# aliabdelkader/FusionTransformer

Measured on AMD Instinct MI355X. Metric: frames/sec fwd+bwd (SemanticKITTI synth), whole job, higher is better.
Workload: dtype f32

## Files before the change

### fusiontransformer_amd/csrc/ftx_spconv.hip

```cpp
#include <cstring>
#include <cstdlib>
#include "ftx_common.h"
#include <rocprim/device/device_scan.hpp>
#include <rocprim/iterator/transform_iterator.hpp>

using namespace ftx;

typedef float f32x16 __attribute__((ext_vector_type(16)));

struct IsValid {
  __host__ __device__ int32_t operator()(int32_t v) const { return v >= 0 ? 1 : 0; }
};

extern "C" size_t ftx_kernel_map_count_workspace_bytes(int64_t n_out, int32_t k) {
  if (n_out <= 0 || k <= 0) return 256;
  size_t bytes = 0;
  const int32_t *in = nullptr;
  int32_t *out = nullptr;
  auto it = rocprim::make_transform_iterator(in, IsValid());
  if (rocprim::exclusive_scan(nullptr, bytes, it, out, 0, (size_t)(n_out * k), rocprim::plus<int32_t>()) != hipSuccess) return 0;
  return bytes + 256;
}

__global__ void koff_kernel(const int32_t *__restrict__ nbr, const int32_t *__restrict__ scan, int64_t n_out, int k, int32_t *__restrict__ koff) {
  int t = blockIdx.x * blockDim.x + threadIdx.x;
  if (t < k) koff[t] = scan[(int64_t)t * n_out];
  if (t == k) {
    int64_t last = (int64_t)k * n_out - 1;
    koff[k] = scan[last] + (nbr[last] >= 0 ? 1 : 0);
  }
}

extern "C" int ftx_kernel_map_count(const int32_t *nbr, int64_t n_out, int32_t k, int32_t *pos, int32_t *koff, void *workspace,
                                    size_t workspace_bytes, void *stream) {
  FTX_REQUIRE(n_out >= 0 && k >= 1, "ftx_kernel_map_count: bad size");
  FTX_REQUIRE(koff, "ftx_kernel_map_count: null koff");
  hipStream_t st = (hipStream_t)stream;
  if (n_out == 0) {
    if (hipMemsetAsync(koff, 0, sizeof(int32_t) * (k + 1), st) != hipSuccess) return check_launch("ftx_kernel_map_count memset");
    return FTX_OK;
  }
  FTX_REQUIRE(nbr && pos && workspace, "ftx_kernel_map_count: null pointer");
  FTX_REQUIRE(n_out * k < 0x7fffffff, "ftx_kernel_map_count: map too large for int32 positions");
  size_t need = ftx_kernel_map_count_workspace_bytes(n_out, k);
  if (workspace_bytes < need) {
    set_error("ftx_kernel_map_count: workspace %zu < required %zu", workspace_bytes, need);
    return FTX_EWORKSPACE;
  }
  size_t bytes = workspace_bytes;
  auto it = rocprim::make_transform_iterator(nbr, IsValid());
  if (rocprim::exclusive_scan(workspace, bytes, it, pos, 0, (size_t)(n_out * k), rocprim::plus<int32_t>(), st) != hipSuccess) {
    set_error("ftx_kernel_map_count: scan failed");
    return FTX_ELAUNCH;
  }
  koff_kernel<<<1, 64, 0, st>>>(nbr, pos, n_out, k, koff);
  return check_launch("ftx_kernel_map_count");
}

__global__ void fill_m1_kernel(int32_t *__restrict__ p, int64_t n) {
  for (int64_t i = blockIdx.x * (int64_t)blockDim.x + threadIdx.x; i < n; i += (int64_t)gridDim.x * blockDim.x) p[i] = -1;
}

__global__ void pairs_scatter_kernel(const int32_t *__restrict__ nbr, int64_t n_out, int64_t n_in, int k, int32_t *__restrict__ pos,
                                     int32_t *__restrict__ pos_t, int32_t *__restrict__ pair_in, int32_t *__restrict__ pair_out,
                                     int64_t cap) {
  const int64_t total = n_out * k;
  for (int64_t e = blockIdx.x * (int64_t)blockDim.x + threadIdx.x; e < total; e += (int64_t)gridDim.x * blockDim.x) {
    int32_t i = nbr[e];
    int32_t p = pos[e];
    if (i >= 0 && i < n_in && p < cap) {
      int kk = (int)(e / n_out);
      int64_t o = e - (int64_t)kk * n_out;
      pair_in[p] = i;
      pair_out[p] = (int32_t)o;
      pos_t[(int64_t)kk * n_in + i] = p;
    } else {
      pos[e] = -1;
    }
  }
}

extern "C" int ftx_kernel_map_pairs(const int32_t *nbr, int64_t n_out, int64_t n_in, int32_t k, int32_t *pos, int32_t *pos_t, int32_t *pair_in,
                                    int32_t *pair_out, int64_t n_pairs, void *stream) {
  FTX_REQUIRE(n_out >= 0 && n_in >= 0 && k >= 1 && n_pairs >= 0, "ftx_kernel_map_pairs: bad size");
  hipStream_t st = (hipStream_t)stream;
  if (n_in > 0) {
    FTX_REQUIRE(pos_t, "ftx_kernel_map_pairs: null pos_t");
    fill_m1_kernel<<<grid_for(n_in * k, 256), 256, 0, st>>>(pos_t, n_in * k);
  }
  if (n_out == 0) return check_launch("ftx_kernel_map_pairs");
  FTX_REQUIRE(nbr && pos && (n_pairs == 0 || (pair_in && pair_out)), "ftx_kernel_map_pairs: null pointer");
  pairs_scatter_kernel<<<grid_for(n_out * k, 256), 256, 0, st>>>(nbr, n_out, n_in, k, pos, pos_t, pair_in, pair_out, n_pairs);
  return check_launch("ftx_kernel_map_pairs");
}

constexpr int BK = 32;
constexpr int AS_STRIDE = 36;
constexpr int TILE_P = 128;

template <int NT, int RT>
__global__ __launch_bounds__(256) void pairs_gemm_kernel(const float *__restrict__ A, int64_t rows_a, const int32_t *__restrict__ gather,
                                                         const float *__restrict__ W, int w_transposed, const int32_t *__restrict__ koff,
                                                         int ca, int co, int kvol, float *__restrict__ tmp, const float *__restrict__ bias,
                                                         int64_t n_dense, const int32_t *__restrict__ scatter, int64_t rows_out) {
  constexpr int TILE = TILE_P * RT;
  constexpr int BN = 32 * NT;
  constexpr int BS_STRIDE = AS_STRIDE;
  constexpr int B_PASSES = NT;
  constexpr int A_PASSES = 4 * RT;

  __shared__ __attribute__((aligned(16))) float As[TILE * AS_STRIDE];
  __shared__ __attribute__((aligned(16))) float Bs[BN * BS_STRIDE];
  __shared__ int s_tile[3];

  const int tid = threadIdx.x;
  if (gather == nullptr) {
    if (tid == 0) {
      int64_t left = n_dense - (int64_t)blockIdx.x * TILE;
      s_tile[0] = left > 0 ? 0 : -1;
      s_tile[1] = blockIdx.x * TILE;
      s_tile[2] = left > TILE ? TILE : (int)left;
    }
  } else if (tid < 64) {
    const int lane0 = tid;
    const int b = blockIdx.x;
    int c = (lane0 < kvol) ? koff[lane0 + 1] - koff[lane0] : 0;
    int nt = (c + TILE - 1) / TILE;
    int incl = nt;
#pragma unroll
    for (int off = 1; off < 64; off <<= 1) {
      int v = __shfl_up(incl, off, 64);
      if (lane0 >= off) incl += v;
    }
    int excl = incl - nt;
    bool mine = (lane0 < kvol) && b >= excl && b < incl;
    unsigned long long m = __ballot(mine);
    if (mine) {
      int t = b - excl;
      int left = c - t * TILE;
      s_tile[0] = lane0;
      s_tile[1] = koff[lane0] + t * TILE;
      s_tile[2] = left > TILE ? TILE : left;
    }
    if (m == 0ull && lane0 == 0) s_tile[0] = -1;
  }
  __syncthreads();
  const int k = s_tile[0];
  if (k < 0) return;
  const int p0 = s_tile[1], cnt = s_tile[2];

  const int wave = tid >> 6, lane = tid & 63;
  const int half = lane >> 5, l31 = lane & 31;
  const int n0 = blockIdx.y * BN;
  const int arow = tid >> 3, acol = (tid & 7) * 4;

  const bool kfull = (ca % BK) == 0;
  int32_t src[A_PASSES];
#pragma unroll
  for (int p = 0; p < A_PASSES; ++p) {
    int r = p * 32 + arow;
    int32_t s = 0;
    if (r < cnt) s = gather ? gather[p0 + r] : p0 + r;
    if (s < 0 || s >= rows_a) s = 0;
    src[p] = s;
  }
  const float *Wk = W + (int64_t)k * ca * co;

  f32x16 acc[RT][NT];
#pragma unroll
  for (int r = 0; r < RT; ++r)
#pragma unroll
    for (int j = 0; j < NT; ++j)
#pragma unroll
      for (int g = 0; g < 16; ++g) acc[r][j][g] = 0.f;

  float4 ra[A_PASSES], rb[B_PASSES];
  auto load_chunk = [&](int c0) {
    if (kfull) {
#pragma unroll
      for (int p = 0; p < A_PASSES; ++p) ra[p] = *(const float4 *)&A[(int64_t)src[p] * ca + c0 + acol];
#pragma unroll
      for (int q = 0; q < B_PASSES; ++q) {
        if (!w_transposed) {
          int kk = ((tid >> 6) << 3) + (tid & 7), n4 = n0 + (q * 8 + ((tid >> 3) & 7)) * 4;
          n4 = n4 + 4 <= co ? n4 : co - 4;
          rb[q] = *(const float4 *)&Wk[(int64_t)(c0 + kk) * co + n4];
        } else {
          int e = q * 256 + tid;
          int nn = n0 + (e >> 3), k4 = (e & 7) * 4;
          nn = nn < co ? nn : co - 1;
          rb[q] = *(const float4 *)&Wk[(int64_t)nn * ca + c0 + k4];
        }
      }
      return;
    }
#pragma unroll
    for (int p = 0; p < A_PASSES; ++p) {
      float4 v = make_float4(0.f, 0.f, 0.f, 0.f);
      if (c0 + acol < ca) v = *(const float4 *)&A[(int64_t)src[p] * ca + c0 + acol];
      ra[p] = v;
    }
#pragma unroll
    for (int q = 0; q < B_PASSES; ++q) {
      float4 v = make_float4(0.f, 0.f, 0.f, 0.f);
      if (!w_transposed) {
        int kk = ((tid >> 6) << 3) + (tid & 7), n4 = (q * 8 + ((tid >> 3) & 7)) * 4;
        if (c0 + kk < ca && n0 + n4 < co) v = *(const float4 *)&Wk[(int64_t)(c0 + kk) * co + n0 + n4];
      } else {
        int e = q * 256 + tid;
        int nn = e >> 3, k4 = (e & 7) * 4;
        if (n0 + nn < co && c0 + k4 < ca) v = *(const float4 *)&Wk[(int64_t)(n0 + nn) * ca + c0 + k4];
      }
      rb[q] = v;
    }
  };
  auto store_chunk = [&]() {
#pragma unroll
    for (int p = 0; p < A_PASSES; ++p) *(float4 *)&As[(p * 32 + arow) * AS_STRIDE + acol] = ra[p];
#pragma unroll
    for (int q = 0; q < B_PASSES; ++q) {
      if (!w_transposed) {
        int kk = ((tid >> 6) << 3) + (tid & 7), n4 = (q * 8 + ((tid >> 3) & 7)) * 4;
        Bs[(n4 + 0) * BS_STRIDE + kk] = rb[q].x;
        Bs[(n4 + 1) * BS_STRIDE + kk] = rb[q].y;
        Bs[(n4 + 2) * BS_STRIDE + kk] = rb[q].z;
        Bs[(n4 + 3) * BS_STRIDE + kk] = rb[q].w;
      } else {
        int e = q * 256 + tid;
        int nn = e >> 3, k4 = (e & 7) * 4;
        *(float4 *)&Bs[nn * BS_STRIDE + k4] = rb[q];
      }
    }
  };

  load_chunk(0);
  for (int c0 = 0; c0 < ca; c0 += BK) {
    store_chunk();
    __syncthreads();
    if (c0 + BK < ca) load_chunk(c0 + BK);
    const float *arow_p = &As[(wave * 32 * RT + l31) * AS_STRIDE + 4 * half];
    const float *brow_p = &Bs[l31 * BS_STRIDE + 4 * half];
    float af[2][RT][4], bf[2][NT][4];
    auto load_frag = [&](int buf, int t) {
#pragma unroll
      for (int r = 0; r < RT; ++r) {
        float4 a = *(const float4 *)(arow_p + r * 32 * AS_STRIDE + 8 * t);
        af[buf][r][0] = a.x; af[buf][r][1] = a.y; af[buf][r][2] = a.z; af[buf][r][3] = a.w;
      }
#pragma unroll
      for (int j = 0; j < NT; ++j) {
        float4 b = *(const float4 *)(brow_p + j * 32 * BS_STRIDE + 8 * t);
        bf[buf][j][0] = b.x; bf[buf][j][1] = b.y; bf[buf][j][2] = b.z; bf[buf][j][3] = b.w;
      }
    };
    load_frag(0, 0);
#pragma unroll
    for (int t = 0; t < BK / 8; ++t) {
      if (t + 1 < BK / 8) load_frag((t + 1) & 1, t + 1);
#pragma unroll
      for (int s = 0; s < 4; ++s)
#pragma unroll
        for (int j = 0; j < NT; ++j)
#pragma unroll
          for (int r = 0; r < RT; ++r)
            acc[r][j] = __builtin_amdgcn_mfma_f32_32x32x2f32(bf[t & 1][j][s], af[t & 1][r][s], acc[r][j], 0, 0, 0);
    }
    __syncthreads();
  }

  const bool nfull = n0 + BN <= co;
#pragma unroll
  for (int r = 0; r < RT; ++r) {
    const int row = wave * 32 * RT + r * 32 + l31;
    int64_t drow = row < cnt ? p0 + row : -1;
    bool zero = false;
    if (gather != nullptr && drow >= 0) {
      const int32_t sidx = gather[drow];
      zero = sidx < 0 || sidx >= rows_a;
    }
    if (scatter != nullptr && drow >= 0) {
      drow = scatter[drow];
      if (drow >= rows_out) drow = -1;
    }
    if (drow >= 0) {
      float *dst = tmp + drow * co;
#pragma unroll
      for (int j = 0; j < NT; ++j)
#pragma unroll
        for (int q = 0; q < 4; ++q) {
          const int col = n0 + j * 32 + 8 * q + 4 * half;
          if (nfull || col < co) {
            float4 v = make_float4(acc[r][j][4 * q], acc[r][j][4 * q + 1], acc[r][j][4 * q + 2], acc[r][j][4 * q + 3]);
            if (zero) v = make_float4(0.f, 0.f, 0.f, 0.f);
            if (bias) {
              const float4 bv = *(const float4 *)&bias[col];
              v.x += bv.x; v.y += bv.y; v.z += bv.z; v.w += bv.w;
            }
            *(float4 *)&dst[col] = v;
          }
        }
    }
  }
}

template <int RT>
static void launch_pairs_gemm(int nt, dim3 grid, hipStream_t st, const float *A, int64_t rows_a, const int32_t *gather, const float *W, int wT,
                              const int32_t *koff, int ca, int co, int kvol, float *tmp, const float *bias, int64_t n_dense,
                              const int32_t *scatter = nullptr, int64_t rows_out = 0) {
  switch (nt) {
    case 1: pairs_gemm_kernel<1, RT><<<grid, 256, 0, st>>>(A, rows_a, gather, W, wT, koff, ca, co, kvol, tmp, bias, n_dense, scatter, rows_out); break;
    case 2: pairs_gemm_kernel<2, RT><<<grid, 256, 0, st>>>(A, rows_a, gather, W, wT, koff, ca, co, kvol, tmp, bias, n_dense, scatter, rows_out); break;
    case 3: pairs_gemm_kernel<3, RT><<<grid, 256, 0, st>>>(A, rows_a, gather, W, wT, koff, ca, co, kvol, tmp, bias, n_dense, scatter, rows_out); break;
    default: pairs_gemm_kernel<4, RT><<<grid, 256, 0, st>>>(A, rows_a, gather, W, wT, koff, ca, co, kvol, tmp, bias, n_dense, scatter, rows_out); break;
  }
}

#include "ftx_lastblock.h"

static int gemm_nt(int co, int64_t row_tiles) {
  int nt = co >= 128 ? 4 : (co + 31) / 32;
  if (co > 128 && co % 96 == 0 && co % 128 != 0) nt = 3;
  if (nt == 4 && row_tiles * ceil_div(co, 128) <= 400) nt = 2;
  return nt;
}

extern "C" int32_t ftx_spconv_gemm_block_cols(int32_t co, int64_t n_pairs, int32_t kvol) {
  if (co < 4 || co % 4 != 0 || n_pairs < 0 || kvol < 0) return -1;
  const int64_t row_tiles = ceil_div(n_pairs, TILE_P) + kvol;
  return 32 * gemm_nt(co, row_tiles);
}


extern "C" int ftx_spconv_pairs_gemm(const float *A, int64_t rows_a, const int32_t *gather, const float *W, int32_t w_transposed,
                                     const int32_t *koff, int64_t n_pairs, int32_t ca, int32_t co, int32_t kvol, float *tmp, void *stream) {
  FTX_REQUIRE(n_pairs >= 0 && rows_a >= 0 && kvol >= 1 && kvol <= 64, "ftx_spconv_pairs_gemm: bad size");
  FTX_REQUIRE(ca >= 4 && ca % 4 == 0 && co >= 4 && co % 4 == 0, "ftx_spconv_pairs_gemm: channels must be multiples of 4 (ca=%d co=%d)", ca, co);
  if (n_pairs == 0) return FTX_OK;
  FTX_REQUIRE(A && gather && W && koff && tmp && rows_a >= 1, "ftx_spconv_pairs_gemm: null pointer or empty operand");
  hipStream_t st = (hipStream_t)stream;
  const unsigned tiles_ub = (unsigned)(ceil_div(n_pairs, TILE_P) + kvol);
  const int nt = gemm_nt(co, tiles_ub);
  dim3 grid(tiles_ub, (unsigned)ceil_div(co, 32 * nt));
  launch_pairs_gemm<1>(nt, grid, st, A, rows_a, gather, W, w_transposed, koff, ca, co, kvol, tmp, nullptr, 0);
  return check_launch("ftx_spconv_pairs_gemm");
}

extern "C" int ftx_spconv_pairs_gemm_scatter(const float *A, int64_t rows_a, const int32_t *gather, const int32_t *scatter, const float *W,
                                             int32_t w_transposed, const int32_t *koff, int64_t n_pairs, int32_t ca, int32_t co, int32_t kvol,
                                             float *out, int64_t rows_out, void *stream) {
  FTX_REQUIRE(n_pairs >= 0 && rows_a >= 0 && rows_out >= 0 && kvol >= 1 && kvol <= 64, "ftx_spconv_pairs_gemm_scatter: bad size");
  FTX_REQUIRE(ca >= 4 && ca % 4 == 0 && co >= 4 && co % 4 == 0, "ftx_spconv_pairs_gemm_scatter: channels must be multiples of 4 (ca=%d co=%d)", ca, co);
  if (n_pairs == 0) return FTX_OK;
  FTX_REQUIRE(A && gather && scatter && W && koff && out && rows_a >= 1, "ftx_spconv_pairs_gemm_scatter: null pointer or empty operand");
  hipStream_t st = (hipStream_t)stream;
  const int nt = gemm_nt(co, ceil_div(n_pairs, TILE_P) + kvol);
  dim3 grid((unsigned)(ceil_div(n_pairs, TILE_P) + kvol), (unsigned)ceil_div(co, 32 * nt));
  launch_pairs_gemm<1>(nt, grid, st, A, rows_a, gather, W, w_transposed, koff, ca, co, kvol, out, nullptr, 0, scatter, rows_out);
  return check_launch("ftx_spconv_pairs_gemm_scatter");
}

extern "C" int ftx_rows_gemm(const float *A, int64_t n, const float *W, int32_t w_transposed, const float *bias, int32_t ca, int32_t co,
                             float *out, void *stream) {
  FTX_REQUIRE(n >= 0, "ftx_rows_gemm: n < 0");
  FTX_REQUIRE(ca >= 4 && ca % 4 == 0 && co >= 4 && co % 4 == 0, "ftx_rows_gemm: channels must be multiples of 4 (ca=%d co=%d)", ca, co);
  if (n == 0) return FTX_OK;
  FTX_REQUIRE(A && W && out, "ftx_rows_gemm: null pointer");
  hipStream_t st = (hipStream_t)stream;
  const int nt = gemm_nt(co, ceil_div(n, TILE_P));
  dim3 grid((unsigned)ceil_div(n, TILE_P), (unsigned)ceil_div(co, 32 * nt));
  launch_pairs_gemm<1>(nt, grid, st, A, n, nullptr, W, w_transposed, nullptr, ca, co, 1, out, bias, n);
  return check_launch("ftx_rows_gemm");
}

template <int KVOL>
__global__ void spconv_reduce_kernel(const float *__restrict__ tmp, const int32_t *__restrict__ pos, int64_t n, int co, int kvol,
                                     float *__restrict__ out) {
  const int cv = co >> 2;
  const int64_t total = n * cv;
  for (int64_t e = blockIdx.x * (int64_t)blockDim.x + threadIdx.x; e < total; e += (int64_t)gridDim.x * blockDim.x) {
    int64_t r = e / cv;
    int j = (int)(e - r * cv) * 4;
    float4 acc = make_float4(0.f, 0.f, 0.f, 0.f);
    if (KVOL > 0) {
      int32_t p[KVOL > 0 ? KVOL : 1];
#pragma unroll
      for (int k = 0; k < KVOL; ++k) p[k] = pos[(int64_t)k * n + r];
#pragma unroll
      for (int k = 0; k < KVOL; ++k) {
        if (p[k] >= 0) {
          float4 v = *(const float4 *)&tmp[(int64_t)p[k] * co + j];
          acc.x += v.x; acc.y += v.y; acc.z += v.z; acc.w += v.w;
        }
      }
    } else {
      for (int k = 0; k < kvol; ++k) {
        int32_t q = pos[(int64_t)k * n + r];
        if (q >= 0) {
          float4 v = *(const float4 *)&tmp[(int64_t)q * co + j];
          acc.x += v.x; acc.y += v.y; acc.z += v.z; acc.w += v.w;
        }
      }
    }
    *(float4 *)&out[r * co + j] = acc;
  }
}

extern "C" int ftx_spconv_reduce(const float *tmp, const int32_t *pos, int64_t n, int32_t co, int32_t kvol, float *out, void *stream) {
  FTX_REQUIRE(n >= 0 && kvol >= 1 && co >= 4 && co % 4 == 0, "ftx_spconv_reduce: bad size");
  if (n == 0) return FTX_OK;
  FTX_REQUIRE(pos && out, "ftx_spconv_reduce: null pointer");
  int64_t work = n * (co / 4);
  int64_t g = ceil_div(work, 256);
  if (g > 8192) g = 8192;
  hipStream_t st = (hipStream_t)stream;
  if (kvol == 27)
    spconv_reduce_kernel<27><<<(unsigned)g, 256, 0, st>>>(tmp, pos, n, co, kvol, out);
  else if (kvol == 8)
    spconv_reduce_kernel<8><<<(unsigned)g, 256, 0, st>>>(tmp, pos, n, co, kvol, out);
  else
    spconv_reduce_kernel<0><<<(unsigned)g, 256, 0, st>>>(tmp, pos, n, co, kvol, out);
  return check_launch("ftx_spconv_reduce");
}

template <int KVOL>
__global__ __launch_bounds__(256) void spconv_reduce_stats_kernel(const float *__restrict__ tmp, const int32_t *__restrict__ pos, int64_t n, int co,
                                                                  int kvol, float *__restrict__ out, double *part, StreamScratch sc) {
  extern __shared__ double sh[];
  const int cv = co >> 2;
  const int RL = 256 / cv;
  const int tid = threadIdx.x;
  const int cg = tid % cv, rl = tid / cv;
  const int64_t rows_per_block = ceil_div(n, (int64_t)gridDim.x);
  const int64_t r0 = (int64_t)blockIdx.x * rows_per_block;
  const int64_t r1 = (r0 + rows_per_block < n) ? r0 + rows_per_block : n;
  double s0[4] = {0, 0, 0, 0}, s1[4] = {0, 0, 0, 0};
  if (rl < RL) {
    const int j = cg * 4;
    for (int64_t r = r0 + rl; r < r1; r += RL) {
      float4 acc = make_float4(0.f, 0.f, 0.f, 0.f);
      if (KVOL > 0) {
        int32_t p[KVOL > 0 ? KVOL : 1];
#pragma unroll
        for (int k = 0; k < KVOL; ++k) p[k] = pos[(int64_t)k * n + r];
#pragma unroll
        for (int k = 0; k < KVOL; ++k) {
          if (p[k] >= 0) {
            float4 v = *(const float4 *)&tmp[(int64_t)p[k] * co + j];
            acc.x += v.x; acc.y += v.y; acc.z += v.z; acc.w += v.w;
          }
        }
      } else {
        for (int k = 0; k < kvol; ++k) {
          int32_t q = pos[(int64_t)k * n + r];
          if (q >= 0) {
            float4 v = *(const float4 *)&tmp[(int64_t)q * co + j];
            acc.x += v.x; acc.y += v.y; acc.z += v.z; acc.w += v.w;
          }
        }
      }
      *(float4 *)&out[r * co + j] = acc;
      s0[0] += (double)acc.x; s1[0] += (double)acc.x * (double)acc.x;
      s0[1] += (double)acc.y; s1[1] += (double)acc.y * (double)acc.y;
      s0[2] += (double)acc.z; s1[2] += (double)acc.z * (double)acc.z;
      s0[3] += (double)acc.w; s1[3] += (double)acc.w * (double)acc.w;
    }
#pragma unroll
    for (int v = 0; v < 4; ++v) {
      sh[(0 * RL + rl) * co + j + v] = s0[v];
      sh[(1 * RL + rl) * co + j + v] = s1[v];
    }
  }
  __syncthreads();
  for (int e = tid; e < 2 * co; e += 256) {
    int which = e / co, col = e - which * co;
    double s = 0;
    for (int q = 0; q < RL; ++q) s += sh[(which * RL + q) * co + col];
    lb_store(&part[((int64_t)blockIdx.x * 2 + which) * co + col], s);
  }
  __syncthreads();
  last_block_totals(part, (int)gridDim.x, co, sc, sh, StoreTotals{part + (int64_t)gridDim.x * 2 * co, co});
}

extern "C" int32_t ftx_spconv_reduce_stats_blocks(int64_t n, int32_t co) {
  if (n <= 0 || co < 4) return 1;
  const int rl = 256 / (co / 4) > 0 ? 256 / (co / 4) : 1;
  int64_t b = ceil_div(n, 2 * rl);
  if (b > 2048) b = 2048;
  return (int32_t)(b < 1 ? 1 : b);
}

extern "C" int ftx_spconv_reduce_stats(const float *tmp, const int32_t *pos, int64_t n, int32_t co, int32_t kvol, float *out, double *part,
                                       int32_t nb, void *stream) {
  FTX_REQUIRE(n >= 1 && kvol >= 1 && co >= 4 && co % 4 == 0 && co <= 512, "ftx_spconv_reduce_stats: bad size (co must be a multiple of 4 in [4, 512])");
  FTX_REQUIRE(pos && out && part, "ftx_spconv_reduce_stats: null pointer");
  FTX_REQUIRE(nb == ftx_spconv_reduce_stats_blocks(n, co), "ftx_spconv_reduce_stats: nb must come from ftx_spconv_reduce_stats_blocks");
  hipStream_t st = (hipStream_t)stream;
  const StreamScratch sc = stream_scratch(st);
  if (!sc.counters) return FTX_ELAUNCH;
  const int rl = 256 / (co / 4);
  const size_t lds = sizeof(double) * 2 * rl * co;
  if (kvol == 27)
    spconv_reduce_stats_kernel<27><<<nb, 256, lds, st>>>(tmp, pos, n, co, kvol, out, part, sc);
  else if (kvol == 8)
    spconv_reduce_stats_kernel<8><<<nb, 256, lds, st>>>(tmp, pos, n, co, kvol, out, part, sc);
  else
    spconv_reduce_stats_kernel<0><<<nb, 256, lds, st>>>(tmp, pos, n, co, kvol, out, part, sc);
  return check_launch("ftx_spconv_reduce_stats");
}

constexpr int WG_BR = 32;
constexpr int WG_ROUND = 1024;

template <int N> struct FragLoad;
template <> struct FragLoad<1> { static __device__ __forceinline__ void ld(const float *p, float (&f)[1]) { f[0] = *p; } };
template <> struct FragLoad<2> { static __device__ __forceinline__ void ld(const float *p, float (&f)[2]) { float2 v = *(const float2 *)p; f[0] = v.x; f[1] = v.y; } };
template <> struct FragLoad<3> { static __device__ __forceinline__ void ld(const float *p, float (&f)[3]) { f[0] = p[0]; f[1] = p[1]; f[2] = p[2]; } };
template <> struct FragLoad<4> { static __device__ __forceinline__ void ld(const float *p, float (&f)[4]) { float4 v = *(const float4 *)p; f[0] = v.x; f[1] = v.y; f[2] = v.z; f[3] = v.w; } };

template <int MI, int NI, int WMG, int WNG>
__global__ __launch_bounds__(256) void pairs_wgrad_kernel(const float *__restrict__ A, int64_t rows_a, const int32_t *__restrict__ idx_a,
                                                          const float *__restrict__ G, int64_t rows_g, const int32_t *__restrict__ idx_g,
                                                          const int32_t *__restrict__ koff, int ca, int cg, int kvol, int tile_len,
                                                          float *__restrict__ part, float *__restrict__ dW, int n_dense) {
  constexpr int TM = 32 * MI * WMG, TN = 32 * NI * WNG, KS = 4 / (WMG * WNG);
  constexpr int STAGE = WG_BR * (TM + TN);
  constexpr int RED = KS > 1 ? MI * NI * 1024 * WMG * WNG : 0;
  constexpr int LDSF = STAGE > RED ? STAGE : RED;
  __shared__ __attribute__((aligned(16))) float lds[LDSF];
  __shared__ int32_t s_ia[WG_ROUND], s_ig[WG_ROUND];
  __shared__ uint8_t s_ok[WG_ROUND];
  __shared__ int s_tile[4];
  __shared__ int s_bad;
  float *As = lds, *Gs = lds + WG_BR * TM;

  const int tid = threadIdx.x, wave = tid >> 6, lane = tid & 63;
  const int half = lane >> 5, l31 = lane & 31;
  const int wq = wave % (WMG * WNG), ks = wave / (WMG * WNG);
  const int wm = wq % WMG, wn = wq / WMG;
  if (tid < 64) {
    const int b = blockIdx.x;
    int c = 0;
    if (tid < kvol) c = koff ? koff[tid + 1] - koff[tid] : n_dense;
    int nt = (c + tile_len - 1) / tile_len;
    int incl = nt;
#pragma unroll
    for (int off = 1; off < 64; off <<= 1) {
      int v = __shfl_up(incl, off, 64);
      if (tid >= off) incl += v;
    }
    int excl = incl - nt;
    bool mine = (tid < kvol) && b >= excl && b < incl;
    unsigned long long msk = __ballot(mine);
    if (mine) {
      int t = b - excl;
      int first = (koff ? koff[tid] : 0) + t * tile_len;
      int left = c - t * tile_len;
      s_tile[0] = tid;
      s_tile[1] = first;
      s_tile[2] = first + (left > tile_len ? tile_len : left);
      s_tile[3] = nt;
    }
    if (msk == 0ull && tid == 0) s_tile[0] = -1;
  }
  __syncthreads();
  const int k = s_tile[0];
  if (k < 0) return;
  const int m0 = blockIdx.y * TM, n0 = blockIdx.z * TN;
  const int lo = s_tile[1], hi = s_tile[2];
  const bool single = s_tile[3] == 1;

  f32x16 acc[MI][NI];
#pragma unroll
  for (int i = 0; i < MI; ++i)
#pragma unroll
    for (int j = 0; j < NI; ++j)
#pragma unroll
      for (int g = 0; g < 16; ++g) acc[i][j][g] = 0.f;

  constexpr int QA = TM / 32, QG = TN / 32;
  float4 ra0[QA], rg0[QG], ra1[QA], rg1[QG];
  int rbase = lo, rend = lo;
  int pra[QA], prg[QG], ca_off[QA], cg_off[QG];
#pragma unroll
  for (int q = 0; q < QA; ++q) {
    int e = q * 256 + tid;
    pra[q] = e / (TM / 4);
    int c = m0 + (e - pra[q] * (TM / 4)) * 4;
    ca_off[q] = c + 4 <= ca ? c : ca - 4;
  }
#pragma unroll
  for (int q = 0; q < QG; ++q) {
    int e = q * 256 + tid;
    prg[q] = e / (TN / 4);
    int c = n0 + (e - prg[q] * (TN / 4)) * 4;
    cg_off[q] = c + 4 <= cg ? c : cg - 4;
  }
  auto load_step = [&](int p0, float4 (&ra)[QA], float4 (&rg)[QG]) {
    const int o = p0 - rbase;
    if (o >= WG_ROUND) return;
    int32_t ia[QA], ig[QG];
#pragma unroll
    for (int q = 0; q < QA; ++q) ia[q] = s_ia[(o + pra[q]) & (WG_ROUND - 1)];
#pragma unroll
    for (int q = 0; q < QG; ++q) ig[q] = s_ig[(o + prg[q]) & (WG_ROUND - 1)];
#pragma unroll
    for (int q = 0; q < QA; ++q) ra[q] = *(const float4 *)(A + ((int64_t)ia[q] * ca + ca_off[q]));
#pragma unroll
    for (int q = 0; q < QG; ++q) rg[q] = *(const float4 *)(G + ((int64_t)ig[q] * cg + cg_off[q]));
  };
  auto store_step = [&](int p0, float4 (&ra)[QA], float4 (&rg)[QG]) {
    if (p0 + WG_BR > rend || s_bad) {
#pragma unroll
      for (int q = 0; q < QA; ++q) {
        const int p = p0 + pra[q];
        if (p >= rend || s_ok[(p - rbase) & (WG_ROUND - 1)] == 0) ra[q] = make_float4(0.f, 0.f, 0.f, 0.f);
      }
#pragma unroll
      for (int q = 0; q < QG; ++q) {
        const int p = p0 + prg[q];
        if (p >= rend || s_ok[(p - rbase) & (WG_ROUND - 1)] == 0) rg[q] = make_float4(0.f, 0.f, 0.f, 0.f);
      }
    }
#pragma unroll
    for (int q = 0; q < QA; ++q) *(float4 *)&As[(q * 256 + tid) * 4] = ra[q];
#pragma unroll
    for (int q = 0; q < QG; ++q) *(float4 *)&Gs[(q * 256 + tid) * 4] = rg[q];
  };
  const float *ap = As + wm * 32 * MI + MI * l31, *gp = Gs + wn * 32 * NI + NI * l31;
  auto mfma_step = [&]() {
    constexpr int ITS = WG_BR / 2 / KS;
    float af[2][MI], gf[2][NI];
    auto frag = [&](int buf, int it) {
      const int kk = 2 * (it * KS + ks) + half;
      FragLoad<MI>::ld(ap + kk * TM, af[buf]);
      FragLoad<NI>::ld(gp + kk * TN, gf[buf]);
    };
    frag(0, 0);
#pragma unroll
    for (int it = 0; it < ITS; ++it) {
      if (it + 1 < ITS) frag((it + 1) & 1, it + 1);
#pragma unroll
      for (int i = 0; i < MI; ++i)
#pragma unroll
        for (int j = 0; j < NI; ++j)
          acc[i][j] = __builtin_amdgcn_mfma_f32_32x32x2f32(gf[it & 1][j], af[it & 1][i], acc[i][j], 0, 0, 0);
    }
  };

  for (rbase = lo; rbase < hi; rbase += WG_ROUND) {
    rend = (rbase + WG_ROUND < hi) ? rbase + WG_ROUND : hi;
    __syncthreads();
    if (tid == 0) s_bad = 0;
    __syncthreads();
    for (int t = tid; t < WG_ROUND; t += 256) {
      int32_t ia = 0, ig = 0;
      uint8_t ok = 0;
      if (t < rend - rbase) {
        ia = idx_a ? idx_a[rbase + t] : rbase + t;
        ig = idx_g ? idx_g[rbase + t] : rbase + t;
        ok = 1;
        if (ia < 0 || ia >= rows_a || ig < 0 || ig >= rows_g) {
          ia = ig = 0;
          ok = 0;
          s_bad = 1;
        }
      }
      s_ia[t] = ia;
      s_ig[t] = ig;
      s_ok[t] = ok;
    }
    __syncthreads();
    load_step(rbase, ra0, rg0);
    load_step(rbase + WG_BR, ra1, rg1);
    for (int p0 = rbase; p0 < rend; p0 += 2 * WG_BR) {
      store_step(p0, ra0, rg0);
      __syncthreads();
      load_step(p0 + 2 * WG_BR, ra0, rg0);
      mfma_step();
      __syncthreads();
      if (p0 + WG_BR >= rend) break;
      store_step(p0 + WG_BR, ra1, rg1);
      __syncthreads();
      load_step(p0 + 3 * WG_BR, ra1, rg1);
      mfma_step();
      __syncthreads();
    }
  }

  if (KS > 1) {
    float *red = lds;
    for (int r = 1; r < KS; ++r) {
      if (ks == r) {
#pragma unroll
        for (int i = 0; i < MI; ++i)
#pragma unroll
          for (int j = 0; j < NI; ++j)
#pragma unroll
            for (int g = 0; g < 16; ++g) red[(((wq * MI + i) * NI + j) * 16 + g) * 64 + lane] = acc[i][j][g];
      }
      __syncthreads();
      if (ks == 0) {
#pragma unroll
        for (int i = 0; i < MI; ++i)
#pragma unroll
          for (int j = 0; j < NI; ++j)
#pragma unroll
            for (int g = 0; g < 16; ++g) acc[i][j][g] += red[(((wq * MI + i) * NI + j) * 16 + g) * 64 + lane];
      }
      __syncthreads();
    }
  }

  if (ks == 0) {
    const int64_t mat = (int64_t)ca * cg;
    float *dst = single ? dW + (int64_t)k * mat : part + (int64_t)blockIdx.x * mat;
    const int ab = m0 + wm * 32 * MI + MI * l31, gb = n0 + wn * 32 * NI;
#pragma unroll
    for (int i = 0; i < MI; ++i) {
      const int row = ab + i;
      if (row < ca) {
#pragma unroll
        for (int q = 0; q < 4; ++q) {
          float v[4 * NI];
#pragma unroll
          for (int e = 0; e < 4; ++e)
#pragma unroll
            for (int j = 0; j < NI; ++j) v[e * NI + j] = acc[i][j][4 * q + e];
          const int col = gb + NI * (8 * q + 4 * half);
#pragma unroll
          for (int t = 0; t < NI; ++t)
            if (col + 4 * t < cg) *(float4 *)&dst[(int64_t)row * cg + col + 4 * t] = make_float4(v[4 * t], v[4 * t + 1], v[4 * t + 2], v[4 * t + 3]);
        }
      }
    }
  }
}

#include "ftx_spconv_wgrad_reduce.h"

struct WgradCfg { int mi, wmg, ni, wng; };
static WgradCfg wgrad_config(int ca, int cg) {
  WgradCfg c;
  if (ca <= 32) { c.mi = 1; c.wmg = 1; }
  else if (ca <= 64) { c.mi = 2; c.wmg = 1; }
  else if (ca % 96 == 0 && ca % 128 != 0) { c.mi = 3; c.wmg = 1; }
  else { c.mi = 2; c.wmg = 2; }
  if (cg <= 32) { c.ni = 1; c.wng = 1; }
  else if (cg <= 64) { c.ni = 2; c.wng = 1; }
  else if (cg % 96 == 0 && cg % 128 != 0) { c.ni = 3; c.wng = 1; }
  else { c.ni = 2; c.wng = 2; }
  if (c.mi == 3 && c.ni == 3) { c.mi = 2; c.wmg = 2; }
  return c;
}

static int wgrad_occ(const WgradCfg &c) {
  static const int occ[4][4] = {{8, 4, 3, 3}, {5, 3, 2, 2}, {4, 2, 1, 2}, {3, 2, 2, 2}};
  auto side = [](int i, int w) { return w == 2 ? 3 : i - 1; };
  return occ[side(c.mi, c.wmg)][side(c.ni, c.wng)];
}
extern "C" int32_t ftx_spconv_wgrad_table_blocks(int32_t mi, int32_t wmg, int32_t ni, int32_t wng) {
  if (!((mi >= 1 && mi <= 3 && wmg == 1) || (mi == 2 && wmg == 2)) || !((ni >= 1 && ni <= 3 && wng == 1) || (ni == 2 && wng == 2))) return -1;
  WgradCfg c{mi, wmg, ni, wng};
  return wgrad_occ(c);
}
extern "C" int32_t ftx_spconv_wgrad_resident_blocks(int32_t ca, int32_t cg) { return wgrad_occ(wgrad_config(ca, cg)); }
constexpr int WGRAD_CUS = 256;

static int wgrad_tile_len(int64_t n_pairs, int ca, int cg, int kvol) {
  const WgradCfg c = wgrad_config(ca, cg);
  const int64_t mn_tiles = ceil_div(ca, 32 * c.mi * c.wmg) * ceil_div(cg, 32 * c.ni * c.wng);
  const int64_t slots = (int64_t)WGRAD_CUS * wgrad_occ(c);
  int64_t len = 256;
  for (int rounds = 1; rounds <= 64; ++rounds) {
    int64_t tiles = (slots * rounds * 15 / 16) / mn_tiles - (kvol + 1) / 2;
    if (tiles < 1) tiles = 1;
    len = ceil_div(ceil_div(n_pairs, tiles), 2 * WG_BR) * 2 * WG_BR;
    if (len <= 4096) break;
  }
  if (len < 256) len = 256;
  return (int)len;
}

static int64_t wgrad_tiles_ub(int64_t n_pairs, int tile_len, int kvol) { return ceil_div(n_pairs, tile_len) + kvol; }

extern "C" size_t ftx_spconv_pairs_wgrad_workspace_bytes(int64_t n_pairs, int32_t ca, int32_t cg, int32_t kvol) {
  if (n_pairs <= 0 || ca <= 0 || cg <= 0 || kvol <= 0) return 256;
  int len = wgrad_tile_len(n_pairs, ca, cg, kvol);
  return sizeof(float) * (size_t)wgrad_tiles_ub(n_pairs, len, kvol) * ca * cg;
}

template <int MI, int WMG>
static void launch_wgrad_n(const WgradCfg &c, dim3 grid, hipStream_t st, const float *A, int64_t rows_a, const int32_t *idx_a, const float *G, int64_t rows_g,
                           const int32_t *idx_g, const int32_t *koff, int ca, int cg, int kvol, int tl, float *part, float *dW, int n_dense) {
  if (c.ni == 1)
    pairs_wgrad_kernel<MI, 1, WMG, 1><<<grid, 256, 0, st>>>(A, rows_a, idx_a, G, rows_g, idx_g, koff, ca, cg, kvol, tl, part, dW, n_dense);
  else if (c.ni == 3)
    pairs_wgrad_kernel<MI, 3, WMG, 1><<<grid, 256, 0, st>>>(A, rows_a, idx_a, G, rows_g, idx_g, koff, ca, cg, kvol, tl, part, dW, n_dense);
  else if (c.wng == 1)
    pairs_wgrad_kernel<MI, 2, WMG, 1><<<grid, 256, 0, st>>>(A, rows_a, idx_a, G, rows_g, idx_g, koff, ca, cg, kvol, tl, part, dW, n_dense);
  else
    pairs_wgrad_kernel<MI, 2, WMG, 2><<<grid, 256, 0, st>>>(A, rows_a, idx_a, G, rows_g, idx_g, koff, ca, cg, kvol, tl, part, dW, n_dense);
}

extern "C" int ftx_spconv_pairs_wgrad(const float *A, int64_t rows_a, const int32_t *idx_a, const float *G, int64_t rows_g, const int32_t *idx_g,
                                      const int32_t *koff, int64_t n_pairs, int32_t ca, int32_t cg, int32_t kvol, float *dW, void *workspace,
                                      size_t workspace_bytes, void *stream) {
  FTX_REQUIRE(n_pairs >= 0 && rows_a >= 0 && rows_g >= 0 && kvol >= 1 && kvol <= 64, "ftx_spconv_pairs_wgrad: bad size");
  FTX_REQUIRE(ca >= 4 && ca % 4 == 0 && cg >= 4 && cg % 4 == 0, "ftx_spconv_pairs_wgrad: channels must be multiples of 4 (ca=%d cg=%d)", ca, cg);
  FTX_REQUIRE(dW, "ftx_spconv_pairs_wgrad: null dW");
  hipStream_t st = (hipStream_t)stream;
  const int64_t mat = (int64_t)ca * cg;
  if (n_pairs == 0) {
    if (hipMemsetAsync(dW, 0, sizeof(float) * kvol * mat, st) != hipSuccess) return check_launch("ftx_spconv_pairs_wgrad memset");
    return FTX_OK;
  }
  FTX_REQUIRE(A && G && rows_a >= 1 && rows_g >= 1, "ftx_spconv_pairs_wgrad: null pointer or empty operand");
  const bool dense = (idx_a == nullptr && idx_g == nullptr && koff == nullptr);
  FTX_REQUIRE(dense || (idx_a && idx_g && koff), "ftx_spconv_pairs_wgrad: idx_a, idx_g and koff must be all set or all null (dense rows)");
  FTX_REQUIRE(!dense || (kvol == 1 && n_pairs <= rows_a && n_pairs <= rows_g), "ftx_spconv_pairs_wgrad: dense mode needs kvol == 1 and n_pairs rows in A and G");
  FTX_REQUIRE(n_pairs < 0x7fffffff, "ftx_spconv_pairs_wgrad: too many pairs");
  const int tile_len = wgrad_tile_len(n_pairs, ca, cg, kvol);
  const int64_t tiles = wgrad_tiles_ub(n_pairs, tile_len, kvol);
  size_t need = sizeof(float) * (size_t)tiles * mat;
  if (!workspace || workspace_bytes < need) {
    set_error("ftx_spconv_pairs_wgrad: workspace %zu < required %zu", workspace_bytes, need);
    return FTX_EWORKSPACE;
  }
  float *part = (float *)workspace;
  const WgradCfg c = wgrad_config(ca, cg);
  dim3 grid((unsigned)tiles, (unsigned)ceil_div(ca, 32 * c.mi * c.wmg), (unsigned)ceil_div(cg, 32 * c.ni * c.wng));
  if (c.mi == 1)
    launch_wgrad_n<1, 1>(c, grid, st, A, rows_a, idx_a, G, rows_g, idx_g, koff, ca, cg, kvol, tile_len, part, dW, (int)n_pairs);
  else if (c.mi == 3)
    launch_wgrad_n<3, 1>(c, grid, st, A, rows_a, idx_a, G, rows_g, idx_g, koff, ca, cg, kvol, tile_len, part, dW, (int)n_pairs);
  else if (c.wmg == 1)
    launch_wgrad_n<2, 1>(c, grid, st, A, rows_a, idx_a, G, rows_g, idx_g, koff, ca, cg, kvol, tile_len, part, dW, (int)n_pairs);
  else
    launch_wgrad_n<2, 2>(c, grid, st, A, rows_a, idx_a, G, rows_g, idx_g, koff, ca, cg, kvol, tile_len, part, dW, (int)n_pairs);
  launch_wgrad_reduce(part, koff, kvol, tile_len, (int)n_pairs, mat, tiles, dW, st);
  return check_launch("ftx_spconv_pairs_wgrad");
}
```

Baseline: 152.0.

## Double-buffer LDS stages in sparse-conv weight-gradient kernel for large tiles

For weight-gradient tile configurations with TM*TN >= 4096, the kernel now allocates two LDS stage buffers and alternates between them. This removes one __syncthreads per step, so the MFMA work on one buffer can overlap the stores into the other. Smaller tiles keep the original single-buffer loop. The cost is doubled LDS use for those tiles, which can lower occupancy, and the buffer handoff depends on the remaining barrier ordering being correct.

```diff
diff --git a/fusiontransformer_amd/csrc/ftx_spconv.hip b/fusiontransformer_amd/csrc/ftx_spconv.hip
--- a/fusiontransformer_amd/csrc/ftx_spconv.hip
+++ b/fusiontransformer_amd/csrc/ftx_spconv.hip
@@ -525,7 +525,8 @@
   constexpr int TM = 32 * MI * WMG, TN = 32 * NI * WNG, KS = 4 / (WMG * WNG);
   constexpr int STAGE = WG_BR * (TM + TN);
   constexpr int RED = KS > 1 ? MI * NI * 1024 * WMG * WNG : 0;
-  constexpr int LDSF = STAGE > RED ? STAGE : RED;
+  constexpr int NBUF = TM * TN >= 4096 ? 2 : 1;
+  constexpr int LDSF = NBUF * STAGE > RED ? NBUF * STAGE : RED;
   __shared__ __attribute__((aligned(16))) float lds[LDSF];
   __shared__ int32_t s_ia[WG_ROUND], s_ig[WG_ROUND];
   __shared__ uint8_t s_ok[WG_ROUND];
@@ -608,7 +609,7 @@
 #pragma unroll
     for (int q = 0; q < QG; ++q) rg[q] = *(const float4 *)(G + ((int64_t)ig[q] * cg + cg_off[q]));
   };
-  auto store_step = [&](int p0, float4 (&ra)[QA], float4 (&rg)[QG]) {
+  auto store_step = [&](int p0, float4 (&ra)[QA], float4 (&rg)[QG], int buf) {
     if (p0 + WG_BR > rend || s_bad) {
 #pragma unroll
       for (int q = 0; q < QA; ++q) {
@@ -622,13 +623,14 @@
       }
     }
 #pragma unroll
-    for (int q = 0; q < QA; ++q) *(float4 *)&As[(q * 256 + tid) * 4] = ra[q];
-#pragma unroll
-    for (int q = 0; q < QG; ++q) *(float4 *)&Gs[(q * 256 + tid) * 4] = rg[q];
+    for (int q = 0; q < QA; ++q) *(float4 *)&As[buf * STAGE + (q * 256 + tid) * 4] = ra[q];
+#pragma unroll
+    for (int q = 0; q < QG; ++q) *(float4 *)&Gs[buf * STAGE + (q * 256 + tid) * 4] = rg[q];
   };
-  const float *ap = As + wm * 32 * MI + MI * l31, *gp = Gs + wn * 32 * NI + NI * l31;
-  auto mfma_step = [&]() {
+  const float *ap0 = As + wm * 32 * MI + MI * l31, *gp0 = Gs + wn * 32 * NI + NI * l31;
+  auto mfma_step = [&](int sbuf) {
     constexpr int ITS = WG_BR / 2 / KS;
+    const float *ap = ap0 + sbuf * STAGE, *gp = gp0 + sbuf * STAGE;
     float af[2][MI], gf[2][NI];
     auto frag = [&](int buf, int it) {
       const int kk = 2 * (it * KS + ks) + half;
@@ -672,17 +674,36 @@
     __syncthreads();
     load_step(rbase, ra0, rg0);
     load_step(rbase + WG_BR, ra1, rg1);
-    for (int p0 = rbase; p0 < rend; p0 += 2 * WG_BR) {
-      store_step(p0, ra0, rg0);
+    if (NBUF == 1) {
+      for (int p0 = rbase; p0 < rend; p0 += 2 * WG_BR) {
+        store_step(p0, ra0, rg0, 0);
+        __syncthreads();
+        load_step(p0 + 2 * WG_BR, ra0, rg0);
+        mfma_step(0);
+        __syncthreads();
+        if (p0 + WG_BR >= rend) break;
+        store_step(p0 + WG_BR, ra1, rg1, 0);
+        __syncthreads();
+        load_step(p0 + 3 * WG_BR, ra1, rg1);
+        mfma_step(0);
+        __syncthreads();
+      }
+    } else {
+      store_step(rbase, ra0, rg0, 0);
       __syncthreads();
-      load_step(p0 + 2 * WG_BR, ra0, rg0);
-      mfma_step();
-      __syncthreads();
-      if (p0 + WG_BR >= rend) break;
-      store_step(p0 + WG_BR, ra1, rg1);
-      __syncthreads();
-      load_step(p0 + 3 * WG_BR, ra1, rg1);
-      mfma_step();
+      load_step(rbase + 2 * WG_BR, ra0, rg0);
+      for (int p0 = rbase; p0 < rend; p0 += 2 * WG_BR) {
+        mfma_step(0);
+        if (p0 + WG_BR >= rend) break;
+        store_step(p0 + WG_BR, ra1, rg1, 1);
+        __syncthreads();
+        load_step(p0 + 3 * WG_BR, ra1, rg1);
+        mfma_step(1);
+        if (p0 + 2 * WG_BR >= rend) break;
+        store_step(p0 + 2 * WG_BR, ra0, rg0, 0);
+        __syncthreads();
+        load_step(p0 + 4 * WG_BR, ra0, rg0);
+      }
       __syncthreads();
     }
   }
```

New measurement: 148.8 (median of 6 runs). 0.979x the previous value.
